# karltan0328/POPE

Hardware: AMD Instinct MI355X
Metric: image-pairs/s (DINOv2-S/14 extract+match, 640x480) (higher is better)
Workload: dtype f16x3 (fp32 operands split hi+lo into f16, 3 MFMAs per product, fp32 accumulate)

## Files before the change

pope_amd/csrc/attention_f16x3.hip:

```cpp
#include "common.h"
#include "kernels.h"
#include <cstdlib>
#include <type_traits>

namespace {

typedef _Float16 f16x4 __attribute__((ext_vector_type(4)));
typedef _Float16 f16x8 __attribute__((ext_vector_type(8)));
typedef short s16x4 __attribute__((ext_vector_type(4)));
typedef __attribute__((address_space(3))) s16x4* lds_s16x4_ptr;

constexpr int HD = 64, KT = 64;
constexpr int WAVES = 8;
constexpr int QB = 32 * WAVES;
constexpr int NT = 64 * WAVES;
constexpr int KST = 72;
constexpr int VST = 96;
constexpr int K_PLANE = KT * KST + 32, V_PLANE = KT * VST + 32;
constexpr size_t X3_ATTN_STAGE_BYTES = size_t(2) * (K_PLANE + V_PLANE) * sizeof(_Float16);
constexpr int OST = 68;
constexpr size_t X3_ATTN_EPI_BYTES = size_t(32) * 8 * OST * sizeof(float);


__device__ __forceinline__ f32x16 mfma_f16(f16x8 a, f16x8 b, f32x16 c) {
    return __builtin_amdgcn_mfma_f32_32x32x16_f16(a, b, c, 0, 0, 0);
}
__device__ __forceinline__ void split4(f32x4 v, f16x4& hi, f16x4& lo) { pope_split4(v, hi, lo); }
__device__ __forceinline__ f16x8 cat(f16x4 a, f16x4 b) { return f16x8{a[0], a[1], a[2], a[3], b[0], b[1], b[2], b[3]}; }
__device__ __forceinline__ float vmax3(float a, float b, float c) {
    float d;
    asm("v_max3_f32 %0, %1, %2, %3" : "=v"(d) : "v"(a), "v"(b), "v"(c));
    return d;
}

template <bool OUT_PLANES>
__global__ __launch_bounds__(NT, 2) void attn_f16x3_kernel(const float* __restrict__ qkv, float* __restrict__ out,
                                                             int N, int heads) {
    extern __shared__ __attribute__((aligned(16))) float smem[];
    _Float16* Kh = reinterpret_cast<_Float16*>(smem);
    _Float16* Kl = Kh + K_PLANE;
    _Float16* Vh = Kl + K_PLANE;
    _Float16* Vl = Vh + V_PLANE;

    const int tid = threadIdx.x, lane = tid & 63, wave = tid >> 6;
    const int r = lane & 31, h = lane >> 5;
    const int n_qb = (N + QB - 1) / QB;
    const int logical = xcd_remap(blockIdx.x, gridDim.x);
    const int bh = logical / n_qb, head = bh % heads, b = bh / heads, q0 = (logical - bh * n_qb) * QB;
    const int D = heads * HD, rs = 3 * D;
    const float* base = qkv + size_t(b) * N * rs;
    const int koff = D + head * HD;

    constexpr float QSCALE = 0.125f * 1.44269504088896340736f;
    f16x8 qh[4], ql[4];
    {
        const int qrow = q0 + wave * 32 + r;
#pragma unroll
        for (int kg = 0; kg < 4; ++kg) {
            f32x4 v0 = {0.f, 0.f, 0.f, 0.f}, v1 = {0.f, 0.f, 0.f, 0.f};
            if (qrow < N) {
                const float* p = base + size_t(qrow) * rs + head * HD + 16 * kg + 8 * h;
                v0 = *reinterpret_cast<const f32x4*>(p);
                v1 = *reinterpret_cast<const f32x4*>(p + 4);
            }
            f16x4 h0, l0, h1, l1;
            split4(v0 * QSCALE, h0, l0);
            split4(v1 * QSCALE, h1, l1);
            qh[kg] = cat(h0, h1);
            ql[kg] = cat(l0, l1);
        }
    }

    const __amdgpu_buffer_rsrc_t rsrc =
        __builtin_amdgcn_make_buffer_rsrc(const_cast<float*>(base), 0, unsigned(N) * unsigned(rs) * 4u, 0x00020000);
    constexpr int RPP = NT / 16, NP = KT / RPP;
    const int srow = tid >> 4, scol = (tid & 15) * 4;
    unsigned kvoff[NP];
#pragma unroll
    for (int i = 0; i < NP; ++i) kvoff[i] = (unsigned(srow + RPP * i) * unsigned(rs) + scol + koff) * 4u;
    const unsigned tile_bytes = unsigned(KT) * unsigned(rs) * 4u, v_delta = unsigned(D) * 4u;
    f32x4 rk[NP], rv[NP];
    auto load_kv = [&](int kt) {
#pragma unroll
        for (int i = 0; i < NP; ++i) {
            rk[i] = __builtin_bit_cast(f32x4, __builtin_amdgcn_raw_buffer_load_b128(rsrc, kvoff[i], kt * tile_bytes, 0));
            rv[i] = __builtin_bit_cast(f32x4, __builtin_amdgcn_raw_buffer_load_b128(rsrc, kvoff[i] + v_delta, kt * tile_bytes, 0));
        }
    };
    auto store_kv = [&]() {
#pragma unroll
        for (int i = 0; i < NP; ++i) {
            f16x4 hi, lo;
            split4(rk[i], hi, lo);
            *reinterpret_cast<f16x4*>(Kh + (srow + RPP * i) * KST + scol) = hi;
            *reinterpret_cast<f16x4*>(Kl + (srow + RPP * i) * KST + scol) = lo;
            split4(rv[i], hi, lo);
            *reinterpret_cast<f16x4*>(Vh + (srow + RPP * i) * VST + scol) = hi;
            *reinterpret_cast<f16x4*>(Vl + (srow + RPP * i) * VST + scol) = lo;
        }
    };

    const int tr_off = (4 * h + ((lane & 15) >> 2)) * VST + 16 * ((lane >> 4) & 1) + 4 * (lane & 3);
    auto vfrag = [&](const _Float16* plane, int u, int s, int dt) {
        const _Float16* p = plane + tr_off + (32 * u + 16 * s) * VST + 32 * dt;
        const s16x4 a = __builtin_amdgcn_ds_read_tr16_b64_v4i16((lds_s16x4_ptr)(p));
        const s16x4 c = __builtin_amdgcn_ds_read_tr16_b64_v4i16((lds_s16x4_ptr)(p + 8 * VST));
        return cat(__builtin_bit_cast(f16x4, a), __builtin_bit_cast(f16x4, c));
    };

    f32x16 o0, o1;
#pragma unroll
    for (int i = 0; i < 16; ++i) { o0[i] = 0.f; o1[i] = 0.f; }
    float m_run = -INFINITY;
    f32x2 l_run = {0.f, 0.f};

    auto tile = [&](int kt, auto last_tag) {
        constexpr bool LAST = decltype(last_tag)::value;
        if (kt) __syncthreads();
        store_kv();
        __syncthreads();
        if constexpr (!LAST) load_kv(kt + 1);

        f32x16 s0, s1;
#pragma unroll
        for (int i = 0; i < 16; ++i) { s0[i] = 0.f; s1[i] = 0.f; }
        const _Float16* kb_h = Kh + r * KST + 8 * h;
        const _Float16* kb_l = Kl + r * KST + 8 * h;
#pragma unroll
        for (int kg = 0; kg < 4; ++kg) {
            const f16x8 k0h = *reinterpret_cast<const f16x8*>(kb_h + 16 * kg);
            const f16x8 k1h = *reinterpret_cast<const f16x8*>(kb_h + 32 * KST + 16 * kg);
            const f16x8 k0l = *reinterpret_cast<const f16x8*>(kb_l + 16 * kg);
            const f16x8 k1l = *reinterpret_cast<const f16x8*>(kb_l + 32 * KST + 16 * kg);
            s0 = mfma_f16(k0l, qh[kg], s0);
            s1 = mfma_f16(k1l, qh[kg], s1);
            s0 = mfma_f16(k0h, ql[kg], s0);
            s1 = mfma_f16(k1h, ql[kg], s1);
            s0 = mfma_f16(k0h, qh[kg], s0);
            s1 = mfma_f16(k1h, qh[kg], s1);
        }
        if constexpr (LAST) {
#pragma unroll
            for (int i = 0; i < 16; ++i) {
                const int key = kt * KT + mfma32_row(i, h);
                if (key >= N) s0[i] = -INFINITY;
                if (key + 32 >= N) s1[i] = -INFINITY;
            }
        }
        asm volatile("s_nop 15\n\ts_nop 3" : "+v"(s0), "+v"(s1));
        float mt = vmax3(s0[0], s1[0], s0[1]);
#pragma unroll
        for (int i = 1; i < 15; ++i) mt = vmax3(mt, s1[i], s0[i + 1]);
        mt = vmax3(mt, s1[15], s1[15]);
        mt = __builtin_fmaxf(mt, __shfl_xor(mt, 32));
        const float m_new = __builtin_fmaxf(m_run, mt);
        if (__any(m_new > m_run)) {
            const float alpha = __builtin_amdgcn_exp2f(m_run - m_new);
            l_run = l_run * alpha;
            o0 *= alpha;
            o1 *= alpha;
        }
        m_run = m_new;
        const float mshift = m_new - 10.0f;
        f32x2 ls = {0.f, 0.f};
#pragma unroll
        for (int i = 0; i < 16; i += 2) {
            s0[i] = __builtin_amdgcn_exp2f(s0[i] - mshift);
            s0[i + 1] = __builtin_amdgcn_exp2f(s0[i + 1] - mshift);
            s1[i] = __builtin_amdgcn_exp2f(s1[i] - mshift);
            s1[i + 1] = __builtin_amdgcn_exp2f(s1[i + 1] - mshift);
            ls += f32x2{s0[i], s0[i + 1]} + f32x2{s1[i], s1[i + 1]};
        }
        l_run += ls;

#pragma unroll
        for (int u = 0; u < 2; ++u)
#pragma unroll
            for (int s = 0; s < 2; ++s) {
                f32x4 p0, p1;
#pragma unroll
                for (int e = 0; e < 4; ++e) {
                    p0[e] = (u ? s1 : s0)[8 * s + e];
                    p1[e] = (u ? s1 : s0)[8 * s + 4 + e];
                }
                f16x4 h0, l0, h1, l1;
                split4(p0, h0, l0);
                split4(p1, h1, l1);
                const f16x8 ph = cat(h0, h1), pl = cat(l0, l1);
                const f16x8 v0h = vfrag(Vh, u, s, 0), v0l = vfrag(Vl, u, s, 0);
                const f16x8 v1h = vfrag(Vh, u, s, 1), v1l = vfrag(Vl, u, s, 1);
                o0 = mfma_f16(v0l, ph, o0);
                o1 = mfma_f16(v1l, ph, o1);
                o0 = mfma_f16(v0h, pl, o0);
                o1 = mfma_f16(v1h, pl, o1);
                o0 = mfma_f16(v0h, ph, o0);
                o1 = mfma_f16(v1h, ph, o1);
            }
    };

    const int nkt = (N + KT - 1) / KT;
    load_kv(0);
    for (int kt = 0; kt + 1 < nkt; ++kt) tile(kt, std::false_type{});
    tile(nkt - 1, std::true_type{});
    __syncthreads();

    const float l_half = l_run[0] + l_run[1];
    const float inv = 1.0f / (l_half + __shfl_xor(l_half, 32));
    float* Os = smem + (wave * 32) * OST;
#pragma unroll
    for (int g4 = 0; g4 < 4; ++g4) {
        f32x4 a, c;
#pragma unroll
        for (int e = 0; e < 4; ++e) { a[e] = o0[4 * g4 + e] * inv; c[e] = o1[4 * g4 + e] * inv; }
        *reinterpret_cast<f32x4*>(&Os[r * OST + 8 * g4 + 4 * h]) = a;
        *reinterpret_cast<f32x4*>(&Os[r * OST + 32 + 8 * g4 + 4 * h]) = c;
    }
    __builtin_amdgcn_wave_barrier();
#pragma unroll
    for (int i = 0; i < 8; ++i) {
        const int lr = (lane >> 4) + 4 * i, c4 = (lane & 15) * 4;
        const int qrow = q0 + wave * 32 + lr;
        const f32x4 v = *reinterpret_cast<const f32x4*>(&Os[lr * OST + c4]);
        if (qrow < N) {
            if constexpr (OUT_PLANES) {
                f16x4 hi, lo;
                split4(v * 8.0f, hi, lo);
                const int col = head * HD + c4;
                _Float16* o = reinterpret_cast<_Float16*>(out) + (size_t(b) * N + qrow) * 2 * D + (col >> 5) * 64 + (col & 31);
                *reinterpret_cast<f16x4*>(o) = hi;
                *reinterpret_cast<f16x4*>(o + 32) = lo;
            } else {
                *reinterpret_cast<f32x4*>(out + (size_t(b) * N + qrow) * D + head * HD + c4) = v;
            }
        }
    }
}


#ifdef ATTN_STAMPS
__device__ unsigned long long g_attn_dbg[32 * 8];
#define ATTN_STAMP(t, slot)                                                                                     \
    do {                                                                                                        \
        if (blockIdx.x == 300 && tid == 0 && (t) < 32) g_attn_dbg[(t) * 8 + (slot)] = __builtin_readcyclecounter(); \
    } while (0)
#else
#define ATTN_STAMP(t, slot) do {} while (0)
#endif
__device__ unsigned long long g_attn_exact_passes;
constexpr int STAGE_H = 2 * (K_PLANE + V_PLANE);
constexpr size_t X3_ATTN_PIPE_BYTES = size_t(3) * STAGE_H * sizeof(_Float16);
static_assert(X3_ATTN_PIPE_BYTES >= X3_ATTN_EPI_BYTES, "epilogue staging fits the stages");

template <bool OUT_PLANES, bool IN_PLANES, bool DIAG = false>
__global__ __launch_bounds__(NT, 2) void attn_f16x3_pipe_kernel(const float* __restrict__ qkv, float* __restrict__ out,
                                                                  int N, int heads) {
    extern __shared__ __attribute__((aligned(16))) float smem[];
    _Float16* lds = reinterpret_cast<_Float16*>(smem);

    const int tid = threadIdx.x, lane = tid & 63, wave = tid >> 6;
    const int r = lane & 31, h = lane >> 5;
    const int n_qb = (N + QB - 1) / QB;
    const int logical = xcd_remap(blockIdx.x, gridDim.x);
    const int bh = logical / n_qb, head = bh % heads, b = bh / heads, q0 = (logical - bh * n_qb) * QB;
    const int D = heads * HD, rs = 3 * D;
    const float* base = qkv + size_t(b) * N * rs;
    const int koff = D + head * HD;

    constexpr float QSCALE = 0.125f * 1.44269504088896340736f * (IN_PLANES ? 0.125f * 0.125f : 1.0f);
    f16x8 qh[4], ql[4];
    {
        const int qrow = q0 + wave * 32 + r;
#pragma unroll
        for (int kg = 0; kg < 4; ++kg) {
            f32x4 v0 = {0.f, 0.f, 0.f, 0.f}, v1 = {0.f, 0.f, 0.f, 0.f};
            if (qrow < N) {
                if constexpr (IN_PLANES) {
                    const _Float16* p = reinterpret_cast<const _Float16*>(base) + size_t(qrow) * 2 * rs +
                                        (head * 2 + (kg >> 1)) * 64 + 16 * (kg & 1) + 8 * h;
                    const f16x8 ph = *reinterpret_cast<const f16x8*>(p), pl = *reinterpret_cast<const f16x8*>(p + 32);
#pragma unroll
                    for (int e = 0; e < 4; ++e) {
                        v0[e] = float(ph[e]) + float(pl[e]);
                        v1[e] = float(ph[4 + e]) + float(pl[4 + e]);
                    }
                } else {
                    const float* p = base + size_t(qrow) * rs + head * HD + 16 * kg + 8 * h;
                    v0 = *reinterpret_cast<const f32x4*>(p);
                    v1 = *reinterpret_cast<const f32x4*>(p + 4);
                }
            }
            f16x4 h0, l0, h1, l1;
            split4(v0 * QSCALE, h0, l0);
            split4(v1 * QSCALE, h1, l1);
            qh[kg] = cat(h0, h1);
            ql[kg] = cat(l0, l1);
        }
    }

    const __amdgpu_buffer_rsrc_t rsrc =
        __builtin_amdgcn_make_buffer_rsrc(const_cast<float*>(base), 0, unsigned(N) * unsigned(rs) * 4u, 0x00020000);
    constexpr int RPP = NT / 16, NP = KT / RPP;
    const int srow = tid >> 4, scol = (tid & 15) * 4;
    unsigned kvoff[NP];
#pragma unroll
    for (int i = 0; i < NP; ++i) kvoff[i] = (unsigned(srow + RPP * i) * unsigned(rs) + scol + koff) * 4u;
    const unsigned tile_bytes = unsigned(KT) * unsigned(rs) * 4u, v_delta = unsigned(D) * 4u;
    f32x4 rk[NP], rv[NP];
    auto load_kv = [&](int kt) {
#pragma unroll
        for (int i = 0; i < NP; ++i) {
            rk[i] = __builtin_bit_cast(f32x4, __builtin_amdgcn_raw_buffer_load_b128(rsrc, kvoff[i], kt * tile_bytes, 0));
            rv[i] = __builtin_bit_cast(f32x4, __builtin_amdgcn_raw_buffer_load_b128(rsrc, kvoff[i] + v_delta, kt * tile_bytes, 0));
        }
    };
    f16x4 skh[NP], skl[NP], svh[NP], svl[NP];
    auto split_kv = [&]() {
#pragma unroll
        for (int i = 0; i < NP; ++i) {
            split4(rk[i], skh[i], skl[i]);
            split4(rv[i], svh[i], svl[i]);
        }
    };
    auto write_k_row = [&](int st, int i) {
        _Float16* S = lds + st * STAGE_H;
        *reinterpret_cast<f16x4*>(S + (srow + RPP * i) * KST + scol) = skh[i];
        *reinterpret_cast<f16x4*>(S + K_PLANE + (srow + RPP * i) * KST + scol) = skl[i];
    };
    auto write_v_row = [&](int st, int i) {
        _Float16* S = lds + st * STAGE_H;
        *reinterpret_cast<f16x4*>(S + 2 * K_PLANE + (srow + RPP * i) * VST + scol) = svh[i];
        *reinterpret_cast<f16x4*>(S + 2 * K_PLANE + V_PLANE + (srow + RPP * i) * VST + scol) = svl[i];
    };
    auto write_kv = [&](int st) {
        _Float16* S = lds + st * STAGE_H;
#pragma unroll
        for (int i = 0; i < NP; ++i) {
            *reinterpret_cast<f16x4*>(S + (srow + RPP * i) * KST + scol) = skh[i];
            *reinterpret_cast<f16x4*>(S + K_PLANE + (srow + RPP * i) * KST + scol) = skl[i];
            *reinterpret_cast<f16x4*>(S + 2 * K_PLANE + (srow + RPP * i) * VST + scol) = svh[i];
            *reinterpret_cast<f16x4*>(S + 2 * K_PLANE + V_PLANE + (srow + RPP * i) * VST + scol) = svl[i];
        }
    };

    typedef __attribute__((ext_vector_type(4))) unsigned u32x4;
    u32x4 pa[4] = {}, pb[4] = {};
    const int pkey = tid >> 3, pp = tid & 7;
    const unsigned pl_off = unsigned(pkey) * unsigned(rs) * 4u + unsigned((D >> 5) + head * 2) * 128u + unsigned(pp) * 16u;
    const unsigned pl_vdelta = unsigned(D >> 5) * 128u;
    auto load_planes = [&](int kt, u32x4 (&st)[4]) {
        if (kt * KT >= N) return;
#pragma unroll
        for (int c = 0; c < 4; ++c)
            st[c] = __builtin_amdgcn_raw_buffer_load_b128(rsrc, pl_off + (c >> 1) * pl_vdelta + (c & 1) * 128u, kt * tile_bytes, 0);
    };
    auto write_chunk = [&](int st, int c, const u32x4 (&regs)[4]) {
        _Float16* S = lds + st * STAGE_H + (c < 2 ? 0 : 2 * K_PLANE) + (pp >> 2) * (c < 2 ? K_PLANE : V_PLANE) +
                      pkey * (c < 2 ? KST : VST) + (c & 1) * 32 + (pp & 3) * 8;
        *reinterpret_cast<u32x4*>(S) = regs[c];
    };

    const int tr_off = (4 * h + ((lane & 15) >> 2)) * VST + 16 * ((lane >> 4) & 1) + 4 * (lane & 3);
    auto vfrag = [&](const _Float16* plane, int u, int s, int dt) {
        const _Float16* p = plane + tr_off + (32 * u + 16 * s) * VST + 32 * dt;
        const s16x4 a = __builtin_amdgcn_ds_read_tr16_b64_v4i16((lds_s16x4_ptr)(p));
        const s16x4 c = __builtin_amdgcn_ds_read_tr16_b64_v4i16((lds_s16x4_ptr)(p + 8 * VST));
        return cat(__builtin_bit_cast(f16x4, a), __builtin_bit_cast(f16x4, c));
    };

    f32x16 o0, o1, sb[2][2];
    using P0 = std::integral_constant<int, 0>;
    using P1 = std::integral_constant<int, 1>;
#pragma unroll
    for (int i = 0; i < 16; ++i) { o0[i] = 0.f; o1[i] = 0.f; }
    f32x2 l_run = {0.f, 0.f};
    f32x16 nref;
#pragma unroll
    for (int i = 0; i < 16; ++i) nref[i] = INFINITY;

    struct KFrag { f16x8 k0h, k0l, k1h, k1l; };
    auto read_kfrag = [&](int st, int kg, KFrag& f) {
        const _Float16* kb_h = lds + st * STAGE_H + r * KST + 8 * h + 16 * kg;
        f.k0h = *reinterpret_cast<const f16x8*>(kb_h);
        f.k0l = *reinterpret_cast<const f16x8*>(kb_h + K_PLANE);
        f.k1h = *reinterpret_cast<const f16x8*>(kb_h + 32 * KST);
        f.k1l = *reinterpret_cast<const f16x8*>(kb_h + K_PLANE + 32 * KST);
    };
    auto qk_step = [&](int kg, int j, const KFrag& f, f32x16& d0, f32x16& d1, auto biased) {
        const f32x16 zero = {};
        const f32x16 c_init = decltype(biased)::value ? nref : zero;
        if (j == 0) d0 = mfma_f16(f.k0l, qh[kg], kg == 0 ? c_init : d0);
        if (j == 1) d1 = mfma_f16(f.k1l, qh[kg], kg == 0 ? c_init : d1);
        if (j == 2) d0 = mfma_f16(f.k0h, ql[kg], d0);
        if (j == 3) d1 = mfma_f16(f.k1h, ql[kg], d1);
        if (j == 4) d0 = mfma_f16(f.k0h, qh[kg], d0);
        if (j == 5) d1 = mfma_f16(f.k1h, qh[kg], d1);
    };
    auto mask_tail = [&](int kt, f32x16& d0, f32x16& d1) {
#pragma unroll
        for (int i = 0; i < 16; ++i) {
            const int key = kt * KT + mfma32_row(i, h);
            if (key >= N) d0[i] = -INFINITY;
            if (key + 32 >= N) d1[i] = -INFINITY;
        }
    };
    constexpr float LAZY_HEADROOM = 8.0f, LAZY_LIMIT_LOG2 = 15.99f;
    f32x2 sm_ls = {0.f, 0.f};
    auto exact_prepare = [&](const f32x16& c0, const f32x16& c1) __attribute__((always_inline)) {
        float mt = vmax3(c0[0], c1[0], c0[1]);
#pragma unroll
        for (int i = 1; i < 15; ++i) mt = vmax3(mt, c1[i], c0[i + 1]);
        mt = __builtin_fmaxf(mt, c1[15]);
        float ma, mb;
        pope_xor32_pair(mt, ma, mb);
        const float ref_old = -nref[0];
        const float ref_new = __builtin_fmaxf(ref_old, __builtin_fmaxf(ma, mb) - LAZY_HEADROOM);
        const float delta = ref_old - ref_new;
        const float alpha = __builtin_amdgcn_exp2f(delta);
#pragma unroll
        for (int i = 0; i < 16; ++i) nref[i] = -ref_new;
        l_run = l_run * alpha;
#pragma unroll
        for (int e = 0; e < 16; ++e) { o0[e] *= alpha; o1[e] *= alpha; }
        return delta;
    };
    auto exp_pair = [&](int i, f32x16& c0, f32x16& c1, auto biased) __attribute__((always_inline)) {
        f32x16& c = i < 8 ? c0 : c1;
        const int e = 2 * (i & 7);
        if constexpr (decltype(biased)::value) {
            c[e] = __builtin_amdgcn_exp2f(c[e]);
            c[e + 1] = __builtin_amdgcn_exp2f(c[e + 1]);
        } else {
            c[e] = __builtin_amdgcn_exp2f(c[e] + nref[0]);
            c[e + 1] = __builtin_amdgcn_exp2f(c[e + 1] + nref[0]);
        }
        float a0 = sm_ls[0], a1 = sm_ls[1];
        a0 += c[e];
        asm volatile("" : "+v"(a0));
        a1 += c[e + 1];
        asm volatile("" : "+v"(a1));
        sm_ls = f32x2{a0, a1};
    };
    auto softmax_slice = [&](int slot, auto ptag) __attribute__((always_inline)) {
        if (slot == 0) sm_ls = f32x2{0.f, 0.f};
        if (slot % 3 != 2)
            exp_pair((slot / 3) * 2 + slot % 3, sb[decltype(ptag)::value][0], sb[decltype(ptag)::value][1], std::true_type{});
    };
    float la_mt = 0.f;
    auto lookahead_slice = [&](int slot, const f32x16& n0, const f32x16& n1) __attribute__((always_inline)) {
        if (slot == 0) la_mt = vmax3(n0[0], n1[0], n0[1]);
        else if (slot < 15) la_mt = vmax3(la_mt, n1[slot], n0[slot + 1]);
        else if (slot == 15) la_mt = __builtin_fmaxf(la_mt, n1[15]);
    };
    auto advance = [&](f32x16& n0, f32x16& n1) __attribute__((always_inline)) {
        if (__builtin_expect(__builtin_amdgcn_ballot_w64(!(la_mt < LAZY_LIMIT_LOG2)) != 0, 0)) {
            if constexpr (DIAG)
                if (lane == 0) (void)__hip_atomic_fetch_add(&g_attn_exact_passes, 1ull, __ATOMIC_RELAXED, __HIP_MEMORY_SCOPE_AGENT);
            float ma, mb;
            pope_xor32_pair(la_mt, ma, mb);
            const float over = __builtin_fmaxf(__builtin_fmaxf(ma, mb) - LAZY_HEADROOM, 0.f);
            const float delta = -over, alpha = __builtin_amdgcn_exp2f(delta);
            const float nr = nref[0] + delta;
#pragma unroll
            for (int i = 0; i < 16; ++i) nref[i] = nr;
            l_run = l_run * alpha;
#pragma unroll
            for (int e = 0; e < 16; ++e) { o0[e] *= alpha; o1[e] *= alpha; }
#pragma unroll
            for (int i = 0; i < 16; ++i) { n0[i] += delta; n1[i] += delta; }
        }
    };
    auto settle = [&]() __attribute__((always_inline)) { l_run += sm_ls; };
    auto phase1 = [&](int st_next, auto ptag) {
        f32x16& n0 = sb[decltype(ptag)::value ^ 1][0];
        f32x16& n1 = sb[decltype(ptag)::value ^ 1][1];
        KFrag kf[2];
        read_kfrag(st_next, 0, kf[0]);
#pragma unroll
        for (int i = 0; i < 24; ++i) {
            const int kg = i / 6, j = i % 6;
            if (j == 0 && kg < 3) read_kfrag(st_next, kg + 1, kf[(kg + 1) & 1]);
            qk_step(kg, j, kf[kg & 1], n0, n1, std::true_type{});
            softmax_slice(i, ptag);
            __builtin_amdgcn_sched_barrier(0);
        }
    };
    auto softmax_only = [&](auto ptag) {
#pragma unroll
        for (int i = 0; i < 24; ++i) softmax_slice(i, ptag);
    };
    auto split_group = [&](int g, int half, f16x4& hi, f16x4& lo, auto ptag) {
        const int u = g >> 1, s2 = g & 1;
        f32x4 pv4;
#pragma unroll
        for (int e = 0; e < 4; ++e) pv4[e] = sb[decltype(ptag)::value][u][8 * s2 + 4 * half + e];
        split4(pv4, hi, lo);
    };
    auto phase2 = [&](int st, int st_write, auto split_tag, const u32x4 (&pregs)[4], auto ptag, auto look_tag) {
        constexpr bool SPLIT_KV = decltype(split_tag)::value;
        constexpr bool LOOK = decltype(look_tag)::value;
        const _Float16* Vh = lds + st * STAGE_H + 2 * K_PLANE;
        const _Float16* Vl = Vh + V_PLANE;
        f16x4 h0[2], l0[2], h1[2], l1[2];
        f16x8 vh[2][2], vl[2];
        split_group(0, 0, h0[0], l0[0], ptag);
        split_group(0, 1, h1[0], l1[0], ptag);
        vh[0][0] = vfrag(Vh, 0, 0, 0); vl[0] = vfrag(Vl, 0, 0, 0);
        vh[0][1] = vfrag(Vh, 0, 0, 1); vl[1] = vfrag(Vl, 0, 0, 1);
        __builtin_amdgcn_sched_barrier(0);
#pragma unroll
        for (int i = 0; i < 24; ++i) {
            const int g = i / 6, j = i % 6, cur = g & 1, nxt = cur ^ 1;
            const int u = (g + 1) >> 1, s2 = (g + 1) & 1;
            if (j == 0 && g < 3) { vh[nxt][0] = vfrag(Vh, u, s2, 0); vh[nxt][1] = vfrag(Vh, u, s2, 1); }
            const f16x8 ph = cat(h0[cur], h1[cur]), pl = cat(l0[cur], l1[cur]);
            if (j == 0) o0 = mfma_f16(vl[0], ph, o0);
            if (j == 1) o1 = mfma_f16(vl[1], ph, o1);
            if (j == 2) o0 = mfma_f16(vh[cur][0], pl, o0);
            if (j == 3) o1 = mfma_f16(vh[cur][1], pl, o1);
            if (j == 4) o0 = mfma_f16(vh[cur][0], ph, o0);
            if (j == 5) o1 = mfma_f16(vh[cur][1], ph, o1);
            if (j == 2 && g < 3) { vl[0] = vfrag(Vl, u, s2, 0); vl[1] = vfrag(Vl, u, s2, 1); }
            if (g < 3) {
                if (j == 1) split_group(g + 1, 0, h0[nxt], l0[nxt], ptag);
                if (j == 3) split_group(g + 1, 1, h1[nxt], l1[nxt], ptag);
            }
            if (LOOK && i % 3 != 1) lookahead_slice(i - (i + 1) / 3, sb[decltype(ptag)::value ^ 1][0], sb[decltype(ptag)::value ^ 1][1]);
            if (SPLIT_KV && j == 5) {
                if constexpr (IN_PLANES) {
                    write_chunk(st_write, g, pregs);
                } else {
                    const int i2 = g >> 1;
                    if (g & 1) { split4(rv[i2], svh[i2], svl[i2]); write_v_row(st_write, i2); }
                    else { split4(rk[i2], skh[i2], skl[i2]); write_k_row(st_write, i2); }
                }
            }
            __builtin_amdgcn_sched_barrier(0);
        }
    };

    const int nkt = (N + KT - 1) / KT;
    if constexpr (IN_PLANES) {
        load_planes(0, pa);
        load_planes(1, pb);
#pragma unroll
        for (int c = 0; c < 4; ++c) write_chunk(0, c, pa);
        load_planes(2, pa);
    } else {
        load_kv(0);
        split_kv();
        write_kv(0);
        if (nkt > 1) load_kv(1);
    }
    __syncthreads();
    {
        KFrag kf;
#pragma unroll
        for (int kg = 0; kg < 4; ++kg) {
            read_kfrag(0, kg, kf);
#pragma unroll
            for (int j = 0; j < 6; ++j) qk_step(kg, j, kf, sb[0][0], sb[0][1], std::false_type{});
        }
    }
    if (nkt == 1) mask_tail(0, sb[0][0], sb[0][1]);
    if constexpr (IN_PLANES) {
#pragma unroll
        for (int c = 0; c < 4; ++c) write_chunk(1, c, pb);
        load_planes(3, pb);
    } else if (nkt > 1) {
        split_kv();
        write_kv(1);
        if (nkt > 2) load_kv(2);
    }
    __syncthreads();
    asm volatile("s_nop 15\n\ts_nop 3" : "+v"(sb[0][0]), "+v"(sb[0][1]));
    exact_prepare(sb[0][0], sb[0][1]);
#pragma unroll
    for (int i = 0; i < 16; ++i) { sb[0][0][i] += nref[0]; sb[0][1][i] += nref[0]; }

    int st_cur = 0, st_next = 1, st_write = 2, t = 0;
    auto rotate = [&]() { const int x = st_cur; st_cur = st_next; st_next = st_write; st_write = x; };
    auto steady = [&](u32x4 (&regs)[4], auto ptag) {
        ATTN_STAMP(t, 0);
        phase1(st_next, ptag);
        settle();
        ATTN_STAMP(t, 1);
        phase2(st_cur, st_write, std::true_type{}, regs, ptag, std::true_type{});
        advance(sb[decltype(ptag)::value ^ 1][0], sb[decltype(ptag)::value ^ 1][1]);
        if constexpr (IN_PLANES) load_planes(t + 4, regs);
        else if (t + 3 < nkt) load_kv(t + 3);
        ATTN_STAMP(t, 2);
        __syncthreads();
        ATTN_STAMP(t, 3);
        rotate();
        ++t;
    };
    while (t + 2 < nkt) {
        steady(pa, P0{});
        if (t + 2 < nkt) steady(pb, P1{});
    }
    auto tail = [&](auto ptag) {
        constexpr int P = decltype(ptag)::value;
        using Q = std::integral_constant<int, P ^ 1>;
        if (t + 1 < nkt) {
            phase1(st_next, ptag);
            mask_tail(t + 1, sb[P ^ 1][0], sb[P ^ 1][1]);
            asm volatile("" : "+v"(sb[P ^ 1][0]), "+v"(sb[P ^ 1][1]));
            settle();
            phase2(st_cur, st_write, std::false_type{}, pa, ptag, std::true_type{});
            advance(sb[P ^ 1][0], sb[P ^ 1][1]);
            rotate();
            ++t;
            softmax_only(Q{});
            settle();
            phase2(st_cur, st_write, std::false_type{}, pa, Q{}, std::false_type{});
        } else {
            softmax_only(ptag);
            settle();
            phase2(st_cur, st_write, std::false_type{}, pa, ptag, std::false_type{});
        }
    };
    if (t & 1) tail(P1{});
    else tail(P0{});
    __syncthreads();

    int tid_e = threadIdx.x;
    asm volatile("" : "+v"(tid_e));
    const int lane_e = tid_e & 63, wave_e = tid_e >> 6, r_e = lane_e & 31, h_e = lane_e >> 5;
    const float l_half = l_run[0] + l_run[1];
    const float inv = (IN_PLANES ? 0.125f : 1.0f) / (l_half + __shfl_xor(l_half, 32));
    float* Os = smem + (wave_e * 32) * OST;
#pragma unroll
    for (int g4 = 0; g4 < 4; ++g4) {
        f32x4 a, c;
#pragma unroll
        for (int e = 0; e < 4; ++e) { a[e] = o0[4 * g4 + e] * inv; c[e] = o1[4 * g4 + e] * inv; }
        *reinterpret_cast<f32x4*>(&Os[r_e * OST + 8 * g4 + 4 * h_e]) = a;
        *reinterpret_cast<f32x4*>(&Os[r_e * OST + 32 + 8 * g4 + 4 * h_e]) = c;
    }
    __builtin_amdgcn_wave_barrier();
#pragma unroll
    for (int i = 0; i < 8; ++i) {
        const int lr = (lane_e >> 4) + 4 * i, c4 = (lane_e & 15) * 4;
        const int qrow = q0 + wave_e * 32 + lr;
        const f32x4 v = *reinterpret_cast<const f32x4*>(&Os[lr * OST + c4]);
        if (qrow < N) {
            if constexpr (OUT_PLANES) {
                f16x4 hi, lo;
                split4(v * 8.0f, hi, lo);
                const int col = head * HD + c4;
                _Float16* o = reinterpret_cast<_Float16*>(out) + (size_t(b) * N + qrow) * 2 * D + (col >> 5) * 64 + (col & 31);
                __builtin_nontemporal_store(hi, reinterpret_cast<f16x4*>(o));
                __builtin_nontemporal_store(lo, reinterpret_cast<f16x4*>(o + 32));
            } else {
                *reinterpret_cast<f32x4*>(out + (size_t(b) * N + qrow) * D + head * HD + c4) = v;
            }
        }
    }
}

}

static_assert(K_PLANES_ACT_SCALE == 8.0f, "attention planes epilogue scale");

template <bool OUT_PLANES>
static int launch_attn_x3(const float* qkv, float* out, int B, int N, int heads, hipStream_t stream) {
    if (B <= 0 || N <= 0 || heads <= 0 || size_t(B) * heads * ((N + QB - 1) / QB) > 0x7fffffffull) return POPE_ERR_ARG;
    if ((reinterpret_cast<uintptr_t>(qkv) & 15) || (reinterpret_cast<uintptr_t>(out) & 15)) return POPE_ERR_ARG;
    if (size_t(N) * 3 * heads * HD * 4 >= (size_t(1) << 32)) return POPE_ERR_ARG;
    const dim3 grid(unsigned((N + QB - 1) / QB) * heads * B);
    static pope_dev_mask lds_ok{0};
    if (!pope_opt_in_lds(attn_f16x3_pipe_kernel<OUT_PLANES, false>, X3_ATTN_PIPE_BYTES, lds_ok)) return POPE_ERR_LAUNCH;
    hipLaunchKernelGGL((attn_f16x3_pipe_kernel<OUT_PLANES, false>), grid, dim3(NT), X3_ATTN_PIPE_BYTES, stream, qkv, out, N, heads);
    return pope_check_launch();
}

#ifdef ATTN_STAMPS
extern "C" int pope_lab_attn_stamps(unsigned long long* host256) {
    return hipMemcpyFromSymbol(host256, HIP_SYMBOL(g_attn_dbg), sizeof(unsigned long long) * 256) == hipSuccess ? 0 : -1;
}
#endif

int pope_launch_attention_f16x3(const float* qkv, float* out, int B, int N, int heads, hipStream_t stream) {
    return launch_attn_x3<false>(qkv, out, B, N, heads, stream);
}
int pope_launch_attention_f16x3_planes_io_diag(const void* qkv_planes, void* out_planes, int B, int N, int heads, long long* exact_passes_host,
                                               hipStream_t stream) {
    if (B <= 0 || N <= 0 || heads <= 0 || ((heads * HD) & 31) || size_t(B) * heads * ((N + QB - 1) / QB) > 0x7fffffffull) return POPE_ERR_ARG;
    if ((reinterpret_cast<uintptr_t>(qkv_planes) & 15) || (reinterpret_cast<uintptr_t>(out_planes) & 15) || !exact_passes_host) return POPE_ERR_ARG;
    if (size_t(N) * 3 * heads * HD * 4 >= (size_t(1) << 32)) return POPE_ERR_ARG;
    const dim3 grid(unsigned((N + QB - 1) / QB) * heads * B);
    static pope_dev_mask lds_ok{0};
    if (!pope_opt_in_lds(attn_f16x3_pipe_kernel<true, true, true>, X3_ATTN_PIPE_BYTES, lds_ok)) return POPE_ERR_LAUNCH;
    unsigned long long v = 0;
    if (hipMemcpyToSymbol(HIP_SYMBOL(g_attn_exact_passes), &v, sizeof(v)) != hipSuccess) return POPE_ERR_LAUNCH;
    hipLaunchKernelGGL((attn_f16x3_pipe_kernel<true, true, true>), grid, dim3(NT), X3_ATTN_PIPE_BYTES, stream,
                       static_cast<const float*>(qkv_planes), static_cast<float*>(out_planes), N, heads);
    if (pope_check_launch() || hipStreamSynchronize(stream) != hipSuccess) return POPE_ERR_LAUNCH;
    if (hipMemcpyFromSymbol(&v, HIP_SYMBOL(g_attn_exact_passes), sizeof(v)) != hipSuccess) return POPE_ERR_LAUNCH;
    *exact_passes_host = (long long)v;
    return POPE_OK;
}
int pope_launch_attention_f16x3_planes_io(const void* qkv_planes, void* out_planes, int B, int N, int heads, hipStream_t stream) {
    if (B <= 0 || N <= 0 || heads <= 0 || ((heads * HD) & 31) || size_t(B) * heads * ((N + QB - 1) / QB) > 0x7fffffffull) return POPE_ERR_ARG;
    if ((reinterpret_cast<uintptr_t>(qkv_planes) & 15) || (reinterpret_cast<uintptr_t>(out_planes) & 15)) return POPE_ERR_ARG;
    if (size_t(N) * 3 * heads * HD * 4 >= (size_t(1) << 32)) return POPE_ERR_ARG;
    const dim3 grid(unsigned((N + QB - 1) / QB) * heads * B);
    static pope_dev_mask lds_ok{0};
    if (!pope_opt_in_lds(attn_f16x3_pipe_kernel<true, true>, X3_ATTN_PIPE_BYTES, lds_ok)) return POPE_ERR_LAUNCH;
    hipLaunchKernelGGL((attn_f16x3_pipe_kernel<true, true>), grid, dim3(NT), X3_ATTN_PIPE_BYTES, stream,
                       static_cast<const float*>(qkv_planes), static_cast<float*>(out_planes), N, heads);
    return pope_check_launch();
}


int pope_launch_attention_f16x3_planes(const float* qkv, void* out_planes, int B, int N, int heads, hipStream_t stream) {
    if ((heads * HD) & 31) return POPE_ERR_ARG;
    return launch_attn_x3<true>(qkv, static_cast<float*>(out_planes), B, N, heads, stream);
}
```

Before: 1473.

## Make planes-IO attention kernel persistent with next-item Q/KV prefetch

```diff
diff --git a/pope_amd/csrc/attention_f16x3.hip b/pope_amd/csrc/attention_f16x3.hip
--- a/pope_amd/csrc/attention_f16x3.hip
+++ b/pope_amd/csrc/attention_f16x3.hip
@@ -241,10 +241,25 @@
 __device__ unsigned long long g_attn_dbg[32 * 8];
 #define ATTN_STAMP(t, slot)                                                                                     \
     do {                                                                                                        \
-        if (blockIdx.x == 300 && tid == 0 && (t) < 32) g_attn_dbg[(t) * 8 + (slot)] = __builtin_readcyclecounter(); \
+        if (blockIdx.x == 100 && tid == 0 && (t) < 32) g_attn_dbg[(t) * 8 + (slot)] = __builtin_readcyclecounter(); \
+    } while (0)
+constexpr int ATTN_ITEM_CAP = 4096;
+__device__ unsigned long long g_attn_items[ATTN_ITEM_CAP * 8];
+#define ATTN_ITEM_STAMP(item, slot)                                                                             \
+    do {                                                                                                        \
+        if (threadIdx.x == 0 && (item) < ATTN_ITEM_CAP) {                                                       \
+            unsigned long long* e_ = g_attn_items + (item) * 8;                                                 \
+            e_[slot] = wall_clock64();                                                                          \
+            if ((slot) == 0) {                                                                                  \
+                e_[4] = (unsigned long long)__builtin_amdgcn_s_getreg((15 << 11) | 20) << 32 |                  \
+                        __builtin_amdgcn_s_getreg((31 << 11) | 4);                                              \
+                e_[5] = blockIdx.x;                                                                             \
+            }                                                                                                   \
+        }                                                                                                       \
     } while (0)
 #else
 #define ATTN_STAMP(t, slot) do {} while (0)
+#define ATTN_ITEM_STAMP(item, slot) do {} while (0)
 #endif
 __device__ unsigned long long g_attn_exact_passes;
 constexpr int STAGE_H = 2 * (K_PLANE + V_PLANE);
@@ -253,41 +268,81 @@
 
 template <bool OUT_PLANES, bool IN_PLANES, bool DIAG = false>
 __global__ __launch_bounds__(NT, 2) void attn_f16x3_pipe_kernel(const float* __restrict__ qkv, float* __restrict__ out,
-                                                                  int N, int heads) {
+                                                                  int N_in, int heads_in, int items_in) {
     extern __shared__ __attribute__((aligned(16))) float smem[];
     _Float16* lds = reinterpret_cast<_Float16*>(smem);
 
-    const int tid = threadIdx.x, lane = tid & 63, wave = tid >> 6;
+    constexpr bool PERSIST = IN_PLANES && !DIAG;
+    int pos = blockIdx.x;
+    const int wave_s = __builtin_amdgcn_readfirstlane(int(threadIdx.x) >> 6);
+    auto thread_index = [&]() {
+        int l;
+        asm volatile("v_mbcnt_lo_u32_b32 %0, -1, 0\n\tv_mbcnt_hi_u32_b32 %0, -1, %0" : "=v"(l));
+        return wave_s * 64 + l;
+    };
+    constexpr float QSCALE = 0.125f * 1.44269504088896340736f * (IN_PLANES ? 0.125f * 0.125f : 1.0f);
+    typedef __attribute__((ext_vector_type(4))) unsigned u32x4;
+    f16x8 qph[4], qpl[4];
+    u32x4 pa[4] = {}, pb[4] = {};
+
+    for (;;) {
+    auto fenced = [](int v) { asm volatile("" : "+s"(v)); return v; };
+    const int N = fenced(N_in), heads = fenced(heads_in), items = fenced(items_in);
+    const int n_qb = (N + QB - 1) / QB;
+    const int D = heads * HD, rs = 3 * D;
+    const int nkt = (N + KT - 1) / KT;
+    struct Item { int logical, head, b, q0; };
+    auto locate = [&](int p) {
+        const int nq = fenced(n_qb), nh = fenced(heads);
+        Item it;
+        it.logical = xcd_remap(p, items);
+        const int bh = it.logical / nq;
+        it.head = bh % nh;
+        it.b = bh / nh;
+        it.q0 = (it.logical - bh * nq) * QB;
+        return it;
+    };
+    auto next_pos = [&]() { return fenced(pos + int(gridDim.x)); };
+    auto planes_rsrc = [&](int b, int head) {
+        const unsigned hoff = unsigned((D >> 5) + head * 2) * 128u;
+        return __builtin_amdgcn_make_buffer_rsrc(reinterpret_cast<char*>(const_cast<float*>(qkv)) + size_t(b) * N * rs * 4 + hoff, 0,
+                                                 unsigned(N) * unsigned(rs) * 4u - hoff, 0x00020000);
+    };
+    const int tid = thread_index();
+    const int lane = tid & 63, wave = tid >> 6;
     const int r = lane & 31, h = lane >> 5;
-    const int n_qb = (N + QB - 1) / QB;
-    const int logical = xcd_remap(blockIdx.x, gridDim.x);
-    const int bh = logical / n_qb, head = bh % heads, b = bh / heads, q0 = (logical - bh * n_qb) * QB;
-    const int D = heads * HD, rs = 3 * D;
-    const float* base = qkv + size_t(b) * N * rs;
-    const int koff = D + head * HD;
-
-    constexpr float QSCALE = 0.125f * 1.44269504088896340736f * (IN_PLANES ? 0.125f * 0.125f : 1.0f);
+    const Item cur = locate(pos);
+
     f16x8 qh[4], ql[4];
-    {
-        const int qrow = q0 + wave * 32 + r;
+    auto load_q_planes = [&](const Item& it) {
+        const int tid_q = thread_index(), lane_q = tid_q & 63;
+        const int qrow = it.q0 + (tid_q >> 6) * 32 + (lane_q & 31);
+        const _Float16* p = reinterpret_cast<const _Float16*>(qkv) + (size_t(it.b) * N + qrow) * 2 * rs + it.head * 128 + 8 * (lane_q >> 5);
+#pragma unroll
+        for (int kg = 0; kg < 4; ++kg) {
+            qph[kg] = f16x8{};
+            qpl[kg] = f16x8{};
+            if (qrow < N) {
+                qph[kg] = *reinterpret_cast<const f16x8*>(p + (kg >> 1) * 64 + 16 * (kg & 1));
+                qpl[kg] = *reinterpret_cast<const f16x8*>(p + (kg >> 1) * 64 + 16 * (kg & 1) + 32);
+            }
+        }
+    };
+    auto make_q = [&](const Item& it) {
+        const int qrow = it.q0 + wave * 32 + r;
 #pragma unroll
         for (int kg = 0; kg < 4; ++kg) {
             f32x4 v0 = {0.f, 0.f, 0.f, 0.f}, v1 = {0.f, 0.f, 0.f, 0.f};
-            if (qrow < N) {
-                if constexpr (IN_PLANES) {
-                    const _Float16* p = reinterpret_cast<const _Float16*>(base) + size_t(qrow) * 2 * rs +
-                                        (head * 2 + (kg >> 1)) * 64 + 16 * (kg & 1) + 8 * h;
-                    const f16x8 ph = *reinterpret_cast<const f16x8*>(p), pl = *reinterpret_cast<const f16x8*>(p + 32);
-#pragma unroll
-                    for (int e = 0; e < 4; ++e) {
-                        v0[e] = float(ph[e]) + float(pl[e]);
-                        v1[e] = float(ph[4 + e]) + float(pl[4 + e]);
-                    }
-                } else {
-                    const float* p = base + size_t(qrow) * rs + head * HD + 16 * kg + 8 * h;
-                    v0 = *reinterpret_cast<const f32x4*>(p);
-                    v1 = *reinterpret_cast<const f32x4*>(p + 4);
+            if constexpr (IN_PLANES) {
+#pragma unroll
+                for (int e = 0; e < 4; ++e) {
+                    v0[e] = float(qph[kg][e]) + float(qpl[kg][e]);
+                    v1[e] = float(qph[kg][4 + e]) + float(qpl[kg][4 + e]);
                 }
+            } else if (qrow < N) {
+                const float* p = qkv + (size_t(it.b) * N + qrow) * rs + it.head * HD + 16 * kg + 8 * h;
+                v0 = *reinterpret_cast<const f32x4*>(p);
+                v1 = *reinterpret_cast<const f32x4*>(p + 4);
             }
             f16x4 h0, l0, h1, l1;
             split4(v0 * QSCALE, h0, l0);
@@ -295,15 +350,13 @@
             qh[kg] = cat(h0, h1);
             ql[kg] = cat(l0, l1);
         }
-    }
-
-    const __amdgpu_buffer_rsrc_t rsrc =
-        __builtin_amdgcn_make_buffer_rsrc(const_cast<float*>(base), 0, unsigned(N) * unsigned(rs) * 4u, 0x00020000);
+    };
+
+    __amdgpu_buffer_rsrc_t rsrc =
+        __builtin_amdgcn_make_buffer_rsrc(const_cast<float*>(qkv), 0, 0u, 0x00020000);
     constexpr int RPP = NT / 16, NP = KT / RPP;
     const int srow = tid >> 4, scol = (tid & 15) * 4;
     unsigned kvoff[NP];
-#pragma unroll
-    for (int i = 0; i < NP; ++i) kvoff[i] = (unsigned(srow + RPP * i) * unsigned(rs) + scol + koff) * 4u;
     const unsigned tile_bytes = unsigned(KT) * unsigned(rs) * 4u, v_delta = unsigned(D) * 4u;
     f32x4 rk[NP], rv[NP];
     auto load_kv = [&](int kt) {
@@ -342,16 +395,19 @@
         }
     };
 
-    typedef __attribute__((ext_vector_type(4))) unsigned u32x4;
-    u32x4 pa[4] = {}, pb[4] = {};
     const int pkey = tid >> 3, pp = tid & 7;
-    const unsigned pl_off = unsigned(pkey) * unsigned(rs) * 4u + unsigned((D >> 5) + head * 2) * 128u + unsigned(pp) * 16u;
+    const unsigned pl_off = unsigned(pkey) * unsigned(rs) * 4u + unsigned(pp) * 16u;
     const unsigned pl_vdelta = unsigned(D >> 5) * 128u;
+    const __amdgpu_buffer_rsrc_t prs = planes_rsrc(cur.b, cur.head);
+    const bool has_next = PERSIST && pos + int(gridDim.x) < items;
+    auto load_tile = [&](__amdgpu_buffer_rsrc_t d, int kt, u32x4 (&st)[4]) {
+#pragma unroll
+        for (int c = 0; c < 4; ++c)
+            st[c] = __builtin_amdgcn_raw_buffer_load_b128(d, pl_off + (c >> 1) * pl_vdelta + (c & 1) * 128u, kt * tile_bytes, 0);
+    };
     auto load_planes = [&](int kt, u32x4 (&st)[4]) {
         if (kt * KT >= N) return;
-#pragma unroll
-        for (int c = 0; c < 4; ++c)
-            st[c] = __builtin_amdgcn_raw_buffer_load_b128(rsrc, pl_off + (c >> 1) * pl_vdelta + (c & 1) * 128u, kt * tile_bytes, 0);
+        load_tile(prs, kt, st);
     };
     auto write_chunk = [&](int st, int c, const u32x4 (&regs)[4]) {
         _Float16* S = lds + st * STAGE_H + (c < 2 ? 0 : 2 * K_PLANE) + (pp >> 2) * (c < 2 ? K_PLANE : V_PLANE) +
@@ -370,12 +426,8 @@
     f32x16 o0, o1, sb[2][2];
     using P0 = std::integral_constant<int, 0>;
     using P1 = std::integral_constant<int, 1>;
-#pragma unroll
-    for (int i = 0; i < 16; ++i) { o0[i] = 0.f; o1[i] = 0.f; }
-    f32x2 l_run = {0.f, 0.f};
+    f32x2 l_run;
     f32x16 nref;
-#pragma unroll
-    for (int i = 0; i < 16; ++i) nref[i] = INFINITY;
 
     struct KFrag { f16x8 k0h, k0l, k1h, k1l; };
     auto read_kfrag = [&](int st, int kg, KFrag& f) {
@@ -538,19 +590,40 @@
         }
     };
 
-    const int nkt = (N + KT - 1) / KT;
+    ATTN_ITEM_STAMP(cur.logical, 0);
+    const bool ahead = pos != int(blockIdx.x);
     if constexpr (IN_PLANES) {
-        load_planes(0, pa);
-        load_planes(1, pb);
+        if (!ahead) load_q_planes(cur);
+    } else {
+        const float* base = qkv + size_t(cur.b) * N * rs;
+        rsrc = __builtin_amdgcn_make_buffer_rsrc(const_cast<float*>(base), 0, unsigned(N) * unsigned(rs) * 4u, 0x00020000);
+#pragma unroll
+        for (int i = 0; i < NP; ++i) kvoff[i] = (unsigned(srow + RPP * i) * unsigned(rs) + scol + D + cur.head * HD) * 4u;
+    }
+#pragma unroll
+    for (int i = 0; i < 16; ++i) { o0[i] = 0.f; o1[i] = 0.f; nref[i] = INFINITY; }
+    l_run = f32x2{0.f, 0.f};
+    sb[1][0] = __builtin_nondeterministic_value(sb[1][0]);
+    sb[1][1] = __builtin_nondeterministic_value(sb[1][1]);
+
+    if constexpr (IN_PLANES) {
+        if (!ahead) {
+            load_planes(0, pa);
+            load_planes(1, pb);
+        }
 #pragma unroll
         for (int c = 0; c < 4; ++c) write_chunk(0, c, pa);
+#pragma unroll
+        for (int c = 0; c < 4; ++c) write_chunk(1, c, pb);
         load_planes(2, pa);
+        load_planes(3, pb);
     } else {
         load_kv(0);
         split_kv();
         write_kv(0);
         if (nkt > 1) load_kv(1);
     }
+    make_q(cur);
     __syncthreads();
     {
         KFrag kf;
@@ -562,20 +635,19 @@
         }
     }
     if (nkt == 1) mask_tail(0, sb[0][0], sb[0][1]);
-    if constexpr (IN_PLANES) {
-#pragma unroll
-        for (int c = 0; c < 4; ++c) write_chunk(1, c, pb);
-        load_planes(3, pb);
-    } else if (nkt > 1) {
-        split_kv();
-        write_kv(1);
-        if (nkt > 2) load_kv(2);
-    }
-    __syncthreads();
+    if constexpr (!IN_PLANES) {
+        if (nkt > 1) {
+            split_kv();
+            write_kv(1);
+            if (nkt > 2) load_kv(2);
+        }
+        __syncthreads();
+    }
     asm volatile("s_nop 15\n\ts_nop 3" : "+v"(sb[0][0]), "+v"(sb[0][1]));
     exact_prepare(sb[0][0], sb[0][1]);
 #pragma unroll
     for (int i = 0; i < 16; ++i) { sb[0][0][i] += nref[0]; sb[0][1][i] += nref[0]; }
+    ATTN_ITEM_STAMP(cur.logical, 1);
 
     int st_cur = 0, st_next = 1, st_write = 2, t = 0;
     auto rotate = [&]() { const int x = st_cur; st_cur = st_next; st_next = st_write; st_write = x; };
@@ -621,10 +693,18 @@
     };
     if (t & 1) tail(P1{});
     else tail(P0{});
+    if constexpr (PERSIST) {
+        const Item nx = locate(has_next ? next_pos() : fenced(pos));
+        load_q_planes(nx);
+        const __amdgpu_buffer_rsrc_t d = planes_rsrc(nx.b, nx.head);
+        load_tile(d, 0, pa);
+        load_tile(d, nkt > 1 ? 1 : 0, pb);
+    }
+    ATTN_ITEM_STAMP(cur.logical, 2);
+    const Item ce = locate(fenced(pos));
     __syncthreads();
 
-    int tid_e = threadIdx.x;
-    asm volatile("" : "+v"(tid_e));
+    const int tid_e = thread_index();
     const int lane_e = tid_e & 63, wave_e = tid_e >> 6, r_e = lane_e & 31, h_e = lane_e >> 5;
     const float l_half = l_run[0] + l_run[1];
     const float inv = (IN_PLANES ? 0.125f : 1.0f) / (l_half + __shfl_xor(l_half, 32));
@@ -641,20 +721,25 @@
 #pragma unroll
     for (int i = 0; i < 8; ++i) {
         const int lr = (lane_e >> 4) + 4 * i, c4 = (lane_e & 15) * 4;
-        const int qrow = q0 + wave_e * 32 + lr;
+        const int qrow = ce.q0 + wave_e * 32 + lr;
         const f32x4 v = *reinterpret_cast<const f32x4*>(&Os[lr * OST + c4]);
         if (qrow < N) {
             if constexpr (OUT_PLANES) {
                 f16x4 hi, lo;
                 split4(v * 8.0f, hi, lo);
-                const int col = head * HD + c4;
-                _Float16* o = reinterpret_cast<_Float16*>(out) + (size_t(b) * N + qrow) * 2 * D + (col >> 5) * 64 + (col & 31);
+                const int col = ce.head * HD + c4;
+                _Float16* o = reinterpret_cast<_Float16*>(out) + (size_t(ce.b) * N + qrow) * 2 * D + (col >> 5) * 64 + (col & 31);
                 __builtin_nontemporal_store(hi, reinterpret_cast<f16x4*>(o));
                 __builtin_nontemporal_store(lo, reinterpret_cast<f16x4*>(o + 32));
             } else {
-                *reinterpret_cast<f32x4*>(out + (size_t(b) * N + qrow) * D + head * HD + c4) = v;
+                *reinterpret_cast<f32x4*>(out + (size_t(ce.b) * N + qrow) * D + ce.head * HD + c4) = v;
             }
         }
+    }
+    ATTN_ITEM_STAMP(ce.logical, 3);
+    if (!has_next) break;
+    __syncthreads();
+    pos += int(gridDim.x);
     }
 }
 
@@ -670,13 +755,21 @@
     const dim3 grid(unsigned((N + QB - 1) / QB) * heads * B);
     static pope_dev_mask lds_ok{0};
     if (!pope_opt_in_lds(attn_f16x3_pipe_kernel<OUT_PLANES, false>, X3_ATTN_PIPE_BYTES, lds_ok)) return POPE_ERR_LAUNCH;
-    hipLaunchKernelGGL((attn_f16x3_pipe_kernel<OUT_PLANES, false>), grid, dim3(NT), X3_ATTN_PIPE_BYTES, stream, qkv, out, N, heads);
+    hipLaunchKernelGGL((attn_f16x3_pipe_kernel<OUT_PLANES, false>), grid, dim3(NT), X3_ATTN_PIPE_BYTES, stream, qkv, out, N, heads,
+                       int(grid.x));
     return pope_check_launch();
 }
 
 #ifdef ATTN_STAMPS
 extern "C" int pope_lab_attn_stamps(unsigned long long* host256) {
     return hipMemcpyFromSymbol(host256, HIP_SYMBOL(g_attn_dbg), sizeof(unsigned long long) * 256) == hipSuccess ? 0 : -1;
+}
+extern "C" int pope_lab_attn_item_stamps(unsigned long long* host, int clear) {
+    if (clear) {
+        static unsigned long long zeros[ATTN_ITEM_CAP * 8];
+        return hipMemcpyToSymbol(HIP_SYMBOL(g_attn_items), zeros, sizeof(zeros)) == hipSuccess ? 0 : -1;
+    }
+    return hipMemcpyFromSymbol(host, HIP_SYMBOL(g_attn_items), sizeof(unsigned long long) * ATTN_ITEM_CAP * 8) == hipSuccess ? 0 : -1;
 }
 #endif
 
@@ -688,13 +781,14 @@
     if (B <= 0 || N <= 0 || heads <= 0 || ((heads * HD) & 31) || size_t(B) * heads * ((N + QB - 1) / QB) > 0x7fffffffull) return POPE_ERR_ARG;
     if ((reinterpret_cast<uintptr_t>(qkv_planes) & 15) || (reinterpret_cast<uintptr_t>(out_planes) & 15) || !exact_passes_host) return POPE_ERR_ARG;
     if (size_t(N) * 3 * heads * HD * 4 >= (size_t(1) << 32)) return POPE_ERR_ARG;
-    const dim3 grid(unsigned((N + QB - 1) / QB) * heads * B);
+    const int items = (N + QB - 1) / QB * heads * B;
+    const dim3 grid{unsigned(items)};
     static pope_dev_mask lds_ok{0};
     if (!pope_opt_in_lds(attn_f16x3_pipe_kernel<true, true, true>, X3_ATTN_PIPE_BYTES, lds_ok)) return POPE_ERR_LAUNCH;
     unsigned long long v = 0;
     if (hipMemcpyToSymbol(HIP_SYMBOL(g_attn_exact_passes), &v, sizeof(v)) != hipSuccess) return POPE_ERR_LAUNCH;
     hipLaunchKernelGGL((attn_f16x3_pipe_kernel<true, true, true>), grid, dim3(NT), X3_ATTN_PIPE_BYTES, stream,
-                       static_cast<const float*>(qkv_planes), static_cast<float*>(out_planes), N, heads);
+                       static_cast<const float*>(qkv_planes), static_cast<float*>(out_planes), N, heads, items);
     if (pope_check_launch() || hipStreamSynchronize(stream) != hipSuccess) return POPE_ERR_LAUNCH;
     if (hipMemcpyFromSymbol(&v, HIP_SYMBOL(g_attn_exact_passes), sizeof(v)) != hipSuccess) return POPE_ERR_LAUNCH;
     *exact_passes_host = (long long)v;
@@ -704,11 +798,12 @@
     if (B <= 0 || N <= 0 || heads <= 0 || ((heads * HD) & 31) || size_t(B) * heads * ((N + QB - 1) / QB) > 0x7fffffffull) return POPE_ERR_ARG;
     if ((reinterpret_cast<uintptr_t>(qkv_planes) & 15) || (reinterpret_cast<uintptr_t>(out_planes) & 15)) return POPE_ERR_ARG;
     if (size_t(N) * 3 * heads * HD * 4 >= (size_t(1) << 32)) return POPE_ERR_ARG;
-    const dim3 grid(unsigned((N + QB - 1) / QB) * heads * B);
+    const int items = (N + QB - 1) / QB * heads * B;
+    const dim3 grid(unsigned(std::min(items, pope_cu_count())));
     static pope_dev_mask lds_ok{0};
     if (!pope_opt_in_lds(attn_f16x3_pipe_kernel<true, true>, X3_ATTN_PIPE_BYTES, lds_ok)) return POPE_ERR_LAUNCH;
     hipLaunchKernelGGL((attn_f16x3_pipe_kernel<true, true>), grid, dim3(NT), X3_ATTN_PIPE_BYTES, stream,
-                       static_cast<const float*>(qkv_planes), static_cast<float*>(out_planes), N, heads);
+                       static_cast<const float*>(qkv_planes), static_cast<float*>(out_planes), N, heads, items);
     return pope_check_launch();
 }
 
```

Result: no change. 1474, median of 3 (+0.1%).
